# Lennart0HU/Master-Thesis-Deep-Reinforcement-Learning-DDPG-in-Home-Energy-Management

Measured on AMD Instinct MI355X. Metric: env-steps/sec, higher is better.
Workload: dtype f32; 1 GPU; 65536 parallel shems_LU1 envs per GPU, Charger98 synthetic train table (4320 rows), 72-step episodes, mode=train; envs_per_gpu=65536, episode_len=72, mode=train

## Files before the change

### master-thesis-deep-reinforcement-learning-ddpg-in-home-energy-management_amd/csrc/shems_policy.hip

```cpp
#include <hip/hip_runtime.h>

#include <cstdlib>
#include <cstdio>
#include <cstring>
#include <type_traits>

#include "shems_env_dev.h"
#include "shems_internal.h"

namespace shems {

typedef float f32x16 __attribute__((ext_vector_type(16)));
typedef float f32x4 __attribute__((ext_vector_type(4)));
typedef float f32x2 __attribute__((ext_vector_type(2)));
template <int N> struct FVec { typedef float type __attribute__((ext_vector_type(N))); };
template <> struct FVec<1> { typedef float type; };
template <int N> __device__ __forceinline__ float fvec_get(const typename FVec<N>::type &v, int i) { return v[i]; }
template <> __device__ __forceinline__ float fvec_get<1>(const float &v, int) { return v; }

constexpr int kIn = 9, kH1 = SHEMS_L1, kH2 = SHEMS_L2, kOut = 2;

template <int NA> __device__ __forceinline__ int act_col(int nbase, int t, int row) { return nbase + 64 * (t >> 1) + 2 * row + (t & 1); }
template <int NA> __device__ __forceinline__ typename FVec<NA>::type act_load_a(const float *row_at_nbase, int li);
template <> __device__ __forceinline__ FVec<4>::type act_load_a<4>(const float *p, int li)
// ... 666 lines not shown
        constexpr int keep0_ = free_keep<RD>(-1);
        asm volatile("s_waitcnt vmcnt(%0)" ::"n"(keep0_) : "memory");
        __builtin_amdgcn_sched_barrier(0);
    }
    constexpr int kFreeKsteps = (kChunks - 1) * (kKC / 2) + (kH1 - (kChunks - 1) * kKC) / 2;
    AVec af_[3];
    BVec bf_[3];
#pragma unroll
    for (int k0 = 0; k0 < 2; ++k0) {
        af_[k0] = act_load_a<NA>(Wf + (2 * k0 + lh) * 128, li);
        bf_[k0] = *reinterpret_cast<const BVec *>(Hc + TM * li + (2 * k0 + lh) * BM);
    }
    __builtin_amdgcn_sched_barrier(0);
    FREE_CHUNK(0, kKC / 2);  PSTAMP(3); FREE_CHUNK(1, kKC / 2);  FREE_CHUNK(2, kKC / 2);  FREE_CHUNK(3, kKC / 2);
    FREE_CHUNK(4, kKC / 2);  FREE_CHUNK(5, kKC / 2);  FREE_CHUNK(6, kKC / 2);  FREE_CHUNK(7, kKC / 2);
    if constexpr (HR < 256) {
        asm volatile("s_waitcnt lgkmcnt(0)\n\ts_barrier" ::: "memory");
        [[maybe_unused]] RowRegs rr;
        if constexpr (PRE2) act_row_load(tp_at, rr);
        L1_PHASE(HR / 32);
        if constexpr (PRE2) tp.nz = noise_draw(A.p, env0 + (tid & (BM - 1)));
        asm volatile("s_waitcnt lgkmcnt(0)\n\ts_barrier" ::: "memory");
        if constexpr (PRE2) {
            act_row_store(rr, tp);
            tailpre_store(w1 + (tid & (BM - 1)) * kPreDw, tp);
        }
#pragma unroll
        for (int k0 = 0; k0 < 2; ++k0) {
            constexpr int Kp = (kChunks / 2) * (kKC / 2);
            af_[(Kp + k0) % 3] = act_load_a<NA>(Wf + ((kChunks / 2) % RD) * kFreeChunkFloats + (2 * k0 + lh) * 128, li);
            bf_[(Kp + k0) % 3] = *reinterpret_cast<const BVec *>(Hc + TM * li + (2 * k0 + lh) * BM);
        }
        __builtin_amdgcn_sched_barrier(0);
    }
    FREE_CHUNK(8, kKC / 2);  FREE_CHUNK(9, kKC / 2);  FREE_CHUNK(10, kKC / 2); FREE_CHUNK(11, kKC / 2);
    FREE_CHUNK(12, kKC / 2); FREE_CHUNK(13, kKC / 2); FREE_CHUNK(14, kKC / 2);
    PSTAMP(4);
    FREE_CHUNK(15, (kH1 - (kChunks - 1) * kKC) / 2);
    PSTAMP(10);

#pragma unroll
    for (int gl = 0; gl < NA / 2; ++gl)
        act_l3_group<TM, TM == 4 ? 4 : 16>(acc + 2 * gl, tl + kH2P, nbase + 64 * gl, li, lh, RED_OF(nbase / 64 + gl));
    __syncthreads();

    PSTAMP(11);
    double reward = 0.0;
    const int64_t i = env0 + tid;
    if (tid < BM && i < A.m) {
        float p0, p1;
        act_finish(tl, {RED_OF(0), RED_OF(1), RED_OF(2), RED_OF(3)}, {RED_OF(4), RED_OF(5), RED_OF(6), RED_OF(7)}, tid, p0, p1);
        reward = act_env_tail<HP>(A, i, p0, p1, learner, goff, A.obs == A.v.obs ? xR + tid * kIn : nullptr, PRE ? xP + tid * kPreDw : PRE2 ? w1 + tid * kPreDw : nullptr, hp, gx);
    }
    PSTAMP(12);
    act_block_reward<NW>(A, reward, Wc, bid);
}
template <int TM, int NW, int RD>
__global__ __launch_bounds__(64 * NW, NW / 4) void k_act(ActArgs A) { k_act_body<TM, NW, RD, 0>(A, nullptr); }
template <int TM, int NW, int RD>
__global__ __launch_bounds__(64 * NW, NW / 4) void k_act_hp(ActArgs A, const shems_group_hparams *hp) { k_act_body<TM, NW, RD, 1>(A, hp); }
template <int TM, int NW, int RD>
__global__ __launch_bounds__(64 * NW, NW / 4) void k_act_x(ActArgs A, const shems_group_hparams *hp, GroupX gx) { k_act_body<TM, NW, RD, 2>(A, hp, gx); }

constexpr int kGChunkFloats = kKC * 64;
constexpr int kGPieces = 4, kGLastPieces = 3;
constexpr int g_pieces(int ch) { return ch > kChunks - 1 ? 0 : ch == kChunks - 1 ? kGLastPieces : kGPieces; }
template <int RD>
constexpr int g_keep(int c)
{
    int n = 0;
    for (int j = c + 2; j <= c + RD - 1; ++j) n += g_pieces(j);
    return n;
}

struct ActSplit {
    unsigned long long *slot;
};
constexpr unsigned long long kSplitEmpty = ~0ull;

template <int TM, int NW, int RD>
constexpr size_t actg_lds_bytes()
{
    return sizeof(float) * (NW * RD * kGChunkFloats + 16 + 256 * 32 * TM + kW1K * 32 * TM + (kTailFloats + 2) +
                            8 * 32 * TM * kOut + 32 * TM * kIn + 32 * TM * kPreDw + 4);
}

__device__ __forceinline__ void g_piece(const char *sbase, uint32_t voff, uint32_t lds_base, int q)
{
    switch (q) {
    case 0: glds16_asm<-2048>(sbase, voff, lds_base); break;
    case 1: glds16_asm<-1024>(sbase, voff, lds_base); break;
    case 2: glds16_asm<0>(sbase, voff, lds_base); break;
    default: glds16_asm<1024>(sbase, voff, lds_base); break;
    }
}

template <int TM, int NW, int NS, int RD, int HP, bool TILED = false>
__device__ __forceinline__ void k_actg_body(const ActArgs &A, const ActSplit &X, const shems_group_hparams *hp, const GroupX gx = GroupX{nullptr, nullptr})
{
    static_assert(NW * NS == 8 && (NW == 4 || NW == 8), "8 column groups per env tile: 8 waves, or two workgroups of 4");
#ifdef SHEMS_STAMP_ACT
#define GSTAMP(i, cond) do { if (threadIdx.x == 0 && (cond)) { reinterpret_cast<unsigned long long *>(A.block_reward)[2*(i)] = __builtin_amdgcn_s_memtime(); reinterpret_cast<unsigned long long *>(A.block_reward)[2*(i)+1] = __builtin_amdgcn_s_memrealtime(); } } while (0)
#else
#define GSTAMP(i, cond)
#endif
    GSTAMP(0, blockIdx.x == 0);
    static_assert(RD >= 2 && RD <= 4 && TM >= 1 && TM <= 2, "ring of 2..4 chunks; relu(layer 1) fully resident (TM <= 2)");
    constexpr int NT_ = 64 * NW, BM = 32 * TM, HR = 256;
    extern __shared__ __attribute__((aligned(16))) char smem[];
    float *Wc = reinterpret_cast<float *>(smem);
    float *Hc = Wc + NW * RD * kGChunkFloats + 16;
    float *xT = Hc + HR * BM;
    float *tl = xT + kW1K * BM;
    float *red = tl + (kTailFloats + 2);
    float *xR = red + 8 * BM * kOut;
    float *xP = xR + BM * kIn;

    const int tid = threadIdx.x;
    const int lane = tid & 63, wave = __builtin_amdgcn_readfirstlane(tid >> 6);
    const int li = lane & 31, lh = lane >> 5;
    int64_t tile = blockIdx.x;
    int half = 0;
    if constexpr (NS == 2) {
        const unsigned b = blockIdx.x, T = gridDim.x >> 1, full = (T >> 3) << 4;
        if (b < full) { tile = (int64_t)(b >> 4) * 8 + (b & 7); half = (b >> 3) & 1; }
        else { tile = (int64_t)(T >> 3) * 8 + ((b - full) >> 1); half = (b - full) & 1; }
    }
    const int64_t env0 = A.m0 + tile * BM;
    const auto [learner, goff, P, s_min, s_max] = act_who(A, env0);
    const int g = half * NW + wave;
    const int nbase = 64 * g;

    const char *W2g = reinterpret_cast<const char *>(P + kOffW2);
    float *Wg = Wc + wave * (RD * kGChunkFloats);
    const uint32_t ring_lds = lds_addr(Wg) + 2 * 1024;
    constexpr size_t kGTlTile = 4 * 64 * 64 * 4, kGTlP = 2 * 64 * 64 * 4;
    const char *gsbase = TILED ? reinterpret_cast<const char *>(A.w2t) + kGTlP + (size_t)g * kGTlTile : W2g + g * 256;
    uint32_t gvoff[kGPieces];
#pragma unroll
    for (int q = 0; q < kGPieces; ++q)
        gvoff[q] = (uint32_t)((4 * q + (lane >> 4)) * (TILED ? 256 : kH2 * 4) + (lane & 15) * 16 - (q - 2) * 1024);
#define G_CHUNK_OFF(chunk) (TILED ? (size_t)((chunk) >> 2) * (8 * kGTlTile) + (size_t)((chunk) & 3) * (kKC * 256) : (size_t)(chunk) * (kKC * kH2 * 4))
#define G_PIECE(chunk, q)                                                                         \
    g_piece(gsbase + G_CHUNK_OFF(chunk), gvoff[q], ring_lds + ((chunk) % RD) * (kGChunkFloats * 4), (q))
    TailPre tp;
    act_pre_index(A, P, env0 + (tid & (BM - 1)), tp);
    ObsRegs<BM, NT_> xr;
    TlRegs tr;
    act_obs_load(A, s_min, s_max, env0, tid, xr);
    constexpr int kL1PerWave = (8 * TM) / NW;
    static_assert(TM == 1 && (kL1PerWave == 1 || kL1PerWave == 2), "k_actg lays layer 1 down for 32-env tiles");
    float wa_[kL1PerWave][kW1K / 2];
    bool wok_[kL1PerWave];
#pragma unroll
    for (int u = 0; u < kL1PerWave; ++u) {
        const int k = 32 * (wave + NW * u) + li;
        wok_[u] = k < kH1;
#pragma unroll
        for (int s2 = 0; s2 < kW1K / 2; ++s2) {
            const int j = 2 * s2 + lh;
            wa_[u][s2] = P[j * kH1 + min(k, kH1 - 1)];
        }
    }
    act_tl_load(P, tid, tr);
    tp.nz = noise_draw(A.p, env0 + (tid & (BM - 1)));
    RowRegs rr;
    act_row_load(act_row_at(A, P, tp), rr);
    act_obs_store<BM, NT_, true>(A, env0, tid, xr, xT, xR);
    act_tl_store(tid, tr, tl);
    asm volatile("s_waitcnt lgkmcnt(0)\n\ts_barrier" ::: "memory");
    GSTAMP(1, blockIdx.x == 0);
#undef L1_A
#define L1_A(s_, j_, g, which) (wok_[which] ? wa_[which][s_] : 0.0f)
    {
#pragma unroll
        for (int ch = 0; ch < RD - 1; ++ch)
#pragma unroll
            for (int q = 0; q < kGPieces; ++q) G_PIECE(ch, q);
        constexpr int kL1Tiles = 8 * TM;
        if constexpr (kL1Tiles / NW >= 2) {
#pragma unroll
            for (int u = 0; u < kL1Tiles / (2 * NW); ++u) {
                const int t0 = wave + 2 * NW * u, g0 = t0 / TM, b0 = t0 % TM, t1 = t0 + NW, g1 = t1 / TM, b1 = t1 % TM;
                L1_TILE2(g0, b0, Hc + (g0 * 32) * BM + TM * li + b0, g1, b1, Hc + (g1 * 32) * BM + TM * li + b1);
            }
        } else {
            const int g0 = wave / TM, b0 = wave % TM;
            L1_TILE(g0, b0, Hc + (g0 * 32) * BM + TM * li + b0);
        }
        act_row_store(rr, tp);
        tailpre_store(xP + (tid & (BM - 1)) * kPreDw, tp);
    }
    asm volatile("s_waitcnt lgkmcnt(0)\n\ts_barrier" ::: "memory");
    GSTAMP(2, blockIdx.x == 0);

    typedef typename FVec<TM>::type BVec;
    f32x16 acc[2][TM];
#pragma unroll
    for (int a = 0; a < 2; ++a)
#pragma unroll
        for (int r = 0; r < 16; ++r) {
            const float bias = tl[act_col<2>(nbase, a, (r & 3) + 8 * (r >> 2) + 4 * lh)];
#pragma unroll
            for (int b = 0; b < TM; ++b) acc[a][b][r] = bias;
        }
    constexpr int kGKsteps = (kChunks - 1) * (kKC / 2) + (kH1 - (kChunks - 1) * kKC) / 2;
    f32x2 af_[3];
    BVec bf_[3];
#define G_KSTEP(c, ks)                                                                                          \
    do {                                                                                                        \
        const int K_ = 8 * (c) + (ks), K2_ = K_ + 2;                                                            \
        if (K2_ < kGKsteps) {                                                                                   \
            const int c2_ = K2_ >> 3, kr_ = 2 * (K2_ & 7) + lh;                                                 \
            af_[K2_ % 3] = *reinterpret_cast<const f32x2 *>(Wg + (c2_ % RD) * kGChunkFloats + kr_ * 64 + 2 * li); \
            bf_[K2_ % 3] = *reinterpret_cast<const BVec *>(Hc + (c2_ * kKC + kr_) * BM + TM * li);              \
        }                                                                                                       \
        _Pragma("unroll") for (int b = 0; b < TM; ++b)                                                          \
            acc[0][b] = __builtin_amdgcn_mfma_f32_32x32x2f32(af_[K_ % 3][0], fvec_get<TM>(bf_[K_ % 3], b), acc[0][b], 0, 0, 0); \
        _Pragma("unroll") for (int b = 0; b < TM; ++b)                                                          \
            acc[1][b] = __builtin_amdgcn_mfma_f32_32x32x2f32(af_[K_ % 3][1], fvec_get<TM>(bf_[K_ % 3], b), acc[1][b], 0, 0, 0); \
        __builtin_amdgcn_sched_group_barrier(0x008, TM, 0);                                                     \
        __builtin_amdgcn_sched_group_barrier(0x100, 1, 0);                                                      \
        __builtin_amdgcn_sched_group_barrier(0x008, TM, 0);                                                     \
        __builtin_amdgcn_sched_group_barrier(0x100, 1, 0);                                                      \
        __builtin_amdgcn_sched_barrier(0);                                                                      \
        if ((ks) < g_pieces((c) + RD - 1)) { G_PIECE((c) + RD - 1, (ks) < kGPieces ? (ks) : 0); __builtin_amdgcn_sched_barrier(0); } \
    } while (0)
#define G_CHUNK(c, NKS)                                                                                         \
    do {                                                                                                        \
        _Pragma("unroll") for (int ks = 0; ks < ((NKS) < 6 ? (NKS) : 6); ++ks) G_KSTEP(c, ks);                  \
        if ((c) + 1 < kChunks) {                                                                                \
            constexpr int keep_ = g_keep<RD>(c);                                                                \
            asm volatile("s_waitcnt vmcnt(%0)" ::"n"(keep_) : "memory");       \
            __builtin_amdgcn_sched_barrier(0);                                                                  \
        }                                                                                                       \
        _Pragma("unroll") for (int ks = 6; ks < (NKS); ++ks) G_KSTEP(c, ks);                                    \
    } while (0)
    {
        constexpr int keep0_ = g_keep<RD>(-1);
        asm volatile("s_waitcnt vmcnt(%0)" ::"n"(keep0_) : "memory");
        __builtin_amdgcn_sched_barrier(0);
    }
#ifdef SHEMS_STAMP_ACT
    if (lane == 0 && blockIdx.x == 0) reinterpret_cast<unsigned long long *>(A.block_reward)[48 + wave] = __builtin_amdgcn_s_memtime();
#endif
#pragma unroll
    for (int k0 = 0; k0 < 2; ++k0) {
        af_[k0] = *reinterpret_cast<const f32x2 *>(Wg + (2 * k0 + lh) * 64 + 2 * li);
        bf_[k0] = *reinterpret_cast<const BVec *>(Hc + (2 * k0 + lh) * BM + TM * li);
    }
    __builtin_amdgcn_sched_barrier(0);
    G_CHUNK(0, kKC / 2);  GSTAMP(3, blockIdx.x == 0); G_CHUNK(1, kKC / 2);  G_CHUNK(2, kKC / 2);  G_CHUNK(3, kKC / 2);
    G_CHUNK(4, kKC / 2);  G_CHUNK(5, kKC / 2);  G_CHUNK(6, kKC / 2);  G_CHUNK(7, kKC / 2);
    G_CHUNK(8, kKC / 2);  G_CHUNK(9, kKC / 2);  G_CHUNK(10, kKC / 2); G_CHUNK(11, kKC / 2);
    G_CHUNK(12, kKC / 2); G_CHUNK(13, kKC / 2); G_CHUNK(14, kKC / 2);
    GSTAMP(4, blockIdx.x == 0);
    G_CHUNK(15, (kH1 - (kChunks - 1) * kKC) / 2);

    GSTAMP(10, blockIdx.x == 0);
#ifdef SHEMS_STAMP_ACT
    if (lane == 0 && blockIdx.x == 0) reinterpret_cast<unsigned long long *>(A.block_reward)[32 + wave] = __builtin_amdgcn_s_memtime();
#endif
    act_l3_group<TM, 0>(acc, tl + kH2P, nbase, li, lh, red + g * (BM * kOut));
    __syncthreads();
    GSTAMP(8, blockIdx.x == 0);

    double reward = 0.0;
    const int64_t i = env0 + tid;
    bool fin = tid < BM && i < A.m;
    float p0 = 0.0f, p1 = 0.0f;
    if (fin) {
        auto red_g = [red](int q) -> const float * { return red + q * (BM * kOut); };
        if constexpr (NS == 1) {
            act_finish(tl, {red_g(0), red_g(1), red_g(2), red_g(3)}, {red_g(4), red_g(5), red_g(6), red_g(7)}, tid, p0, p1);
        } else {
            const float *const mine4[4] = {red_g(4 * half), red_g(4 * half + 1), red_g(4 * half + 2), red_g(4 * half + 3)};
            float m0 = act_half_sum(mine4, tid, 0), m1 = act_half_sum(mine4, tid, 1);
            unsigned long long mine = ((unsigned long long)__float_as_uint(m1) << 32) | __float_as_uint(m0);
            if (mine == kSplitEmpty) { mine = 0x7FC000007FC00000ull; m0 = m1 = __uint_as_float(0x7FC00000u); }
            unsigned long long *slot = X.slot + tile * BM + tid;
            const unsigned long long got = __hip_atomic_exchange(slot, mine, __ATOMIC_RELAXED, __HIP_MEMORY_SCOPE_AGENT);
            if (got == kSplitEmpty) fin = false;
            else __hip_atomic_store(slot, kSplitEmpty, __ATOMIC_RELAXED, __HIP_MEMORY_SCOPE_AGENT);
            const float o0 = __uint_as_float((uint32_t)got), o1 = __uint_as_float((uint32_t)(got >> 32));
            p0 = act_out(tl, 0, half == 0 ? m0 : o0, half == 0 ? o0 : m0);
            p1 = act_out(tl, 1, half == 0 ? m1 : o1, half == 0 ? o1 : m1);
        }
    }
    GSTAMP(9, blockIdx.x == 0);
    GSTAMP(11, tile == 0 && fin);
    if (fin) reward = act_env_tail<HP>(A, i, p0, p1, learner, goff, A.obs == A.v.obs ? xR + tid * kIn : nullptr, xP + tid * kPreDw, hp, gx);
    GSTAMP(12, tile == 0 && fin);
    if constexpr (NS == 1) act_block_reward<NW>(A, reward, Wc, tile);
}
template <int TM, int NW, int NS, int RD>
__global__ __launch_bounds__(64 * NW) void k_actg(ActArgs A, ActSplit X) { k_actg_body<TM, NW, NS, RD, 0>(A, X, nullptr); }
template <int TM, int NW, int NS, int RD>
__global__ __launch_bounds__(64 * NW) void k_actg_hp(ActArgs A, ActSplit X, const shems_group_hparams *hp) { k_actg_body<TM, NW, NS, RD, 1>(A, X, hp); }
template <int TM, int NW, int NS, int RD>
__global__ __launch_bounds__(64 * NW) void k_actg_x(ActArgs A, ActSplit X, const shems_group_hparams *hp, GroupX gx) { k_actg_body<TM, NW, NS, RD, 2>(A, X, hp, gx); }
template <int TM, int NW, int NS, int RD>
__global__ __launch_bounds__(64 * NW) void k_actg_t(ActArgs A, ActSplit X) { k_actg_body<TM, NW, NS, RD, 0, true>(A, X, nullptr); }

constexpr int k2CR = 4, k2RD = 4, k2CF = k2CR * 128;
constexpr int k2NCH = (kH1 + k2CR - 1) / k2CR;
constexpr int k2_pieces(int ch) { return ch < 0 || ch >= k2NCH ? 0 : ch == k2NCH - 1 ? (kH1 - (k2NCH - 1) * k2CR + 1) / 2 : k2CR / 2; }
constexpr size_t act2_lds_bytes()
{
    return sizeof(float) * (4 * k2RD * k2CF + 16 + 128 * 64 + kW1K * 64 + (kTailFloats + 2) + 64 * kPreDw + 4);
}

__device__ __forceinline__ void k2_piece(const char *sbase, uint32_t voff, uint32_t lds_base, int q)
{
    if (q == 0) glds16_asm<-1024>(sbase, voff, lds_base); else glds16_asm<0>(sbase, voff, lds_base);
}

constexpr size_t k2TlTile = 4 * 64 * 64 * 4, k2TlP = 2 * 64 * 64 * 4;
template <bool TILED> constexpr size_t k2_chunk_off(int ch)
{
    return TILED ? (size_t)(ch >> 4) * (8 * k2TlTile) + (size_t)(ch & 15) * (k2CR * 256) : (size_t)ch * (k2CR * kH2 * 4);
}
template <int HP, bool TILED = false>
__device__ __forceinline__ void k_act2_body(const ActArgs &A, const shems_group_hparams *hp, const GroupX gx = GroupX{nullptr, nullptr})
{
    constexpr int TM = 2, BM = 64, NA = 4, NT_ = 256, HR = 128;
    extern __shared__ __attribute__((aligned(16))) char smem[];
    float *Wc = reinterpret_cast<float *>(smem);
    float *Hc = Wc + 4 * k2RD * k2CF + 16;
    float *xT = Hc + HR * BM;
    float *tl = xT + kW1K * BM;
    float *xP = tl + (kTailFloats + 2);
    const int tid = threadIdx.x;
    const int lane = tid & 63, wave = __builtin_amdgcn_readfirstlane(tid >> 6);
    const int li = lane & 31, lh = lane >> 5;
    int64_t bid = blockIdx.x;
    if (A.gcount > 1 && (gridDim.x & 7) == 0) bid = (int64_t)(blockIdx.x & 7) * (gridDim.x >> 3) + (blockIdx.x >> 3);
    const int64_t env0 = A.m0 + bid * BM;
    const auto [learner, goff, P, s_min, s_max] = act_who(A, env0);
    const int nbase = 128 * wave;

    const char *W2g = reinterpret_cast<const char *>(P + kOffW2);
    float *Wf = Wc + wave * (k2RD * k2CF);
    const uint32_t ring_lds = lds_addr(Wf) + 1024;
    const char *wsbase = TILED ? reinterpret_cast<const char *>(A.w2t) + k2TlP + (size_t)wave * (2 * k2TlTile) : W2g + wave * 512;
    uint32_t wvoff[2];
#pragma unroll
    for (int q = 0; q < 2; ++q)
        wvoff[q] = TILED ? (uint32_t)(((lane & 31) >> 4) * k2TlTile + (lane >> 5) * 256 + (lane & 15) * 16 + q * 512 - (q - 1) * 1024)
                         : (uint32_t)((lane >> 5) * (kH2 * 4) + (lane & 31) * 16 + q * (2 * kH2 * 4) - (q - 1) * 1024);
#define K2_PIECE(chunk, q) k2_piece(wsbase + k2_chunk_off<TILED>(chunk), wvoff[q], ring_lds + ((chunk) % k2RD) * (k2CF * 4), (q))
    TailPre tp;
    act_pre_index(A, P, env0 + (tid & (BM - 1)), tp);
    ObsRegs<BM, NT_> xr;
    TlRegs tr;
    act_obs_load(A, s_min, s_max, env0, tid, xr);
    act_tl_load(P, tid, tr);
#define K2_L1_LOAD(gbase, a0_, a1_, kA_, kB_)                                                     \
    _Pragma("unroll") for (int s_ = 0; s_ < kW1K / 2; ++s_) {                                     \
        const int j_ = 2 * s_ + lh;                                                               \
        a0_[s_] = P[j_ * kH1 + min(kA_, kH1 - 1)];                                                \
        a1_[s_] = P[j_ * kH1 + min(kB_, kH1 - 1)];                                                \
    }
    const int t0 = wave, t1 = wave + 4;
    const int kA0 = 32 * (t0 >> 1) + li, kB0 = 32 * (t1 >> 1) + li;
    float wa0[kW1K / 2], wb0[kW1K / 2];
    K2_L1_LOAD(0, wa0, wb0, kA0, kB0)
    tp.nz = noise_draw(A.p, env0 + (tid & (BM - 1)));
    RowRegs rr;
    act_row_load(act_row_at(A, P, tp), rr);
    act_obs_store<BM, NT_, false>(A, env0, tid, xr, xT, nullptr);
    act_tl_store(tid, tr, tl);
    asm volatile("s_waitcnt lgkmcnt(0)\n\ts_barrier" ::: "memory");
#pragma unroll
    for (int ch = 0; ch < k2RD - 1; ++ch)
#pragma unroll
        for (int q = 0; q < 2; ++q) K2_PIECE(ch, q);

#define K2_L1_PHASE(gbase, a0_, a1_)                                                              \
    do {                                                                                          \
        const int gA_ = (gbase) + (t0 >> 1), bA_ = t0 & 1, gB_ = (gbase) + (t1 >> 1), bB_ = t1 & 1; \
        float c0_[kW1K / 2], c1_[kW1K / 2], z0_[kW1K / 2], z1_[kW1K / 2];                         \
        _Pragma("unroll") for (int s_ = 0; s_ < kW1K / 2; ++s_) {                                 \
            const int j_ = 2 * s_ + lh;                                                           \
            c0_[s_] = xT[j_ * BM + TM * li + bA_];                                                \
            c1_[s_] = xT[j_ * BM + TM * li + bB_];                                                \
            z0_[s_] = 32 * gA_ + li < kH1 ? a0_[s_] : 0.0f;                                       \
            z1_[s_] = 32 * gB_ + li < kH1 ? a1_[s_] : 0.0f;                                       \
        }                                                                                         \
        f32x16 u0_, u1_;                                                                          \
        asm volatile("s_nop 1\n\t"                                                                \
                     "v_mfma_f32_32x32x2_f32 %0, %2, %7, 0\n\t"                                   \
                     "v_mfma_f32_32x32x2_f32 %1, %12, %17, 0\n\t"                                 \
                     "v_mfma_f32_32x32x2_f32 %0, %3, %8, %0\n\t"                                  \
                     "v_mfma_f32_32x32x2_f32 %1, %13, %18, %1\n\t"                                \
                     "v_mfma_f32_32x32x2_f32 %0, %4, %9, %0\n\t"                                  \
                     "v_mfma_f32_32x32x2_f32 %1, %14, %19, %1\n\t"                                \
                     "v_mfma_f32_32x32x2_f32 %0, %5, %10, %0\n\t"                                 \
                     "v_mfma_f32_32x32x2_f32 %1, %15, %20, %1\n\t"                                \
                     "v_mfma_f32_32x32x2_f32 %0, %6, %11, %0\n\t"                                 \
                     "v_mfma_f32_32x32x2_f32 %1, %16, %21, %1\n\t"                                \
                     "s_nop 15\n\ts_nop 7"                                                        \
                     : "=&v"(u0_), "=&v"(u1_)                                                     \
                     : "v"(z0_[0]), "v"(z0_[1]), "v"(z0_[2]), "v"(z0_[3]), "v"(z0_[4]),           \
                       "v"(c0_[0]), "v"(c0_[1]), "v"(c0_[2]), "v"(c0_[3]), "v"(c0_[4]),           \
                       "v"(z1_[0]), "v"(z1_[1]), "v"(z1_[2]), "v"(z1_[3]), "v"(z1_[4]),           \
                       "v"(c1_[0]), "v"(c1_[1]), "v"(c1_[2]), "v"(c1_[3]), "v"(c1_[4]));          \
        float *d0_ = Hc + ((gA_ * 32) % HR) * BM + TM * li + bA_, *d1_ = Hc + ((gB_ * 32) % HR) * BM + TM * li + bB_; \
        _Pragma("unroll") for (int r_ = 0; r_ < 16; ++r_) {                                       \
            d0_[((r_ & 3) + 8 * (r_ >> 2) + 4 * lh) * BM] = fmaxf(u0_[r_], 0.0f);                 \
            d1_[((r_ & 3) + 8 * (r_ >> 2) + 4 * lh) * BM] = fmaxf(u1_[r_], 0.0f);                 \
        }                                                                                         \
    } while (0)
    K2_L1_PHASE(0, wa0, wb0);
    float wa1[kW1K / 2], wb1[kW1K / 2];
    {
        const int kA1 = 128 + kA0, kB1 = 128 + kB0;
        K2_L1_LOAD(4, wa1, wb1, kA1, kB1)
    }
    act_row_store(rr, tp);
    tailpre_store(xP + (tid & (BM - 1)) * kPreDw, tp);
    asm volatile("s_waitcnt lgkmcnt(0)\n\ts_barrier" ::: "memory");

    typedef FVec<NA>::type AVec;
    typedef FVec<TM>::type BVec;
    f32x16 acc[NA][TM];
#pragma unroll
    for (int a = 0; a < NA; ++a)
#pragma unroll
        for (int r = 0; r < 16; ++r) {
            const float bias = tl[act_col<NA>(nbase, a, (r & 3) + 8 * (r >> 2) + 4 * lh)];
#pragma unroll
            for (int b = 0; b < TM; ++b) acc[a][b][r] = bias;
        }
    constexpr int kKsteps = kH1 / 2;
    AVec af_[3];
    BVec bf_[3];
#define K2_KSTEP(K)                                                                                             \
    do {                                                                                                        \
        constexpr int K2_ = (K) + 2, c2_ = K2_ >> 1, klim_ = (K) < 64 ? 64 : kKsteps;                           \
        if (K2_ < klim_) {                                                                                      \
            if ((K2_ & 1) == 0) {                                                                               \
                asm volatile("s_waitcnt vmcnt(%0)" ::"n"(k2_pieces(c2_ + 1)) : "memory");                       \
                __builtin_amdgcn_sched_barrier(0);                                                              \
            }                                                                                                   \
            const int kr_ = 2 * (K2_ & 1) + lh;                                                                 \
            af_[K2_ % 3] = act_load_a<NA>(Wf + (c2_ % k2RD) * k2CF + kr_ * 128, li);                            \
            bf_[K2_ % 3] = *reinterpret_cast<const BVec *>(Hc + ((2 * K2_) % HR + lh) * BM + TM * li);          \
        }                                                                                                       \
        _Pragma("unroll") for (int a = 0; a < NA; ++a)                                                          \
            _Pragma("unroll") for (int b = 0; b < TM; ++b)                                                      \
                acc[a][b] = __builtin_amdgcn_mfma_f32_32x32x2f32(fvec_get<NA>(af_[(K) % 3], a), fvec_get<TM>(bf_[(K) % 3], b), acc[a][b], 0, 0, 0); \
        __builtin_amdgcn_sched_group_barrier(0x008, 2, 0);                                                      \
        __builtin_amdgcn_sched_group_barrier(0x100, 1, 0);                                                      \
        __builtin_amdgcn_sched_group_barrier(0x008, 2, 0);                                                      \
        __builtin_amdgcn_sched_group_barrier(0x100, 1, 0);                                                      \
        __builtin_amdgcn_sched_barrier(0);                                                                      \
        if (((K) & 1) < k2_pieces(((K) >> 1) + k2RD - 1)) { K2_PIECE(((K) >> 1) + k2RD - 1, (K) & 1); __builtin_amdgcn_sched_barrier(0); } \
    } while (0)
#define K2_K4(K) K2_KSTEP(K); K2_KSTEP((K) + 1); K2_KSTEP((K) + 2); K2_KSTEP((K) + 3)
#define K2_K16(K) K2_K4(K); K2_K4((K) + 4); K2_K4((K) + 8); K2_K4((K) + 12)
    asm volatile("s_waitcnt vmcnt(%0)" ::"n"(k2_pieces(1) + k2_pieces(2)) : "memory");
    __builtin_amdgcn_sched_barrier(0);
#pragma unroll
    for (int k0 = 0; k0 < 2; ++k0) {
        af_[k0] = act_load_a<NA>(Wf + (2 * k0 + lh) * 128, li);
        bf_[k0] = *reinterpret_cast<const BVec *>(Hc + (2 * k0 + lh) * BM + TM * li);
    }
    __builtin_amdgcn_sched_barrier(0);
    K2_K16(0); K2_K16(16); K2_K16(32); K2_K16(48);
    asm volatile("s_waitcnt lgkmcnt(0)\n\ts_barrier" ::: "memory");
    K2_L1_PHASE(4, wa1, wb1);
    asm volatile("s_waitcnt lgkmcnt(0)\n\ts_barrier" ::: "memory");
    asm volatile("s_waitcnt vmcnt(%0)" ::"n"(k2_pieces(33) + k2_pieces(34)) : "memory");
    __builtin_amdgcn_sched_barrier(0);
#pragma unroll
    for (int k0 = 0; k0 < 2; ++k0) {
        af_[(64 + k0) % 3] = act_load_a<NA>(Wf + ((32 + (k0 >> 1)) % k2RD) * k2CF + (2 * (k0 & 1) + lh) * 128, li);
        bf_[(64 + k0) % 3] = *reinterpret_cast<const BVec *>(Hc + (2 * k0 + lh) * BM + TM * li);
    }
    __builtin_amdgcn_sched_barrier(0);
    K2_K16(64); K2_K16(80); K2_K16(96); K2_K4(112); K2_K4(116); K2_K4(120); K2_KSTEP(124);

#pragma unroll
    for (int gl = 0; gl < 2; ++gl) act_l3_group<TM, 0>(acc + 2 * gl, tl + kH2P, nbase + 64 * gl, li, lh, Wf + gl * (BM * kOut));
    __syncthreads();
    double reward = 0.0;
    const int64_t i = env0 + tid;
    if (tid < BM && i < A.m) {
        auto red_g = [Wc](int g) -> const float * { return Wc + (g >> 1) * (k2RD * k2CF) + (g & 1) * (BM * kOut); };
        float p0, p1;
        act_finish(tl, {red_g(0), red_g(1), red_g(2), red_g(3)}, {red_g(4), red_g(5), red_g(6), red_g(7)}, tid, p0, p1);
        reward = act_env_tail<HP>(A, i, p0, p1, learner, goff, nullptr, xP + tid * kPreDw, hp, gx);
    }
    act_block_reward<4>(A, reward, Hc, bid);
}
__global__ __launch_bounds__(256, 2) void k_act2(ActArgs A) { k_act2_body<0>(A, nullptr); }
__global__ __launch_bounds__(256, 2) void k_act2_hp(ActArgs A, const shems_group_hparams *hp) { k_act2_body<1>(A, hp); }
__global__ __launch_bounds__(256, 2) void k_act2_x(ActArgs A, const shems_group_hparams *hp, GroupX gx) { k_act2_body<2>(A, hp, gx); }
__global__ __launch_bounds__(256, 2) void k_act2_t(ActArgs A) { k_act2_body<0, true>(A, nullptr); }

template <class... Lead>
struct ActKernels {
    typedef void (*Plain)(Lead...);
    typedef void (*WithHp)(Lead..., const shems_group_hparams *);
    typedef void (*WithX)(Lead..., const shems_group_hparams *, GroupX);
    Plain plain; WithHp with_hp; WithX with_x;
    std::atomic<uint64_t> optin[3];
    char what_attr[3][48], what_launch[3][32];

    ActKernels(const char *name, Plain k, WithHp k_hp, WithX k_x) : plain(k), with_hp(k_hp), with_x(k_x), optin{}
    {
        static const char *const suffix[3] = {"", "_hp", "_x"};
        for (int v = 0; v < 3; ++v) {
            snprintf(what_attr[v], sizeof what_attr[v], "hipFuncSetAttribute(%s%s)", name, suffix[v]);
            snprintf(what_launch[v], sizeof what_launch[v], "%s%s launch", name, suffix[v]);
        }
    }
    int launch(dim3 grid, dim3 block, size_t lds, hipStream_t st, const shems_group_hparams *hp, const GroupX *gx, const Lead &...lead)
    {
        const int v = gx ? 2 : hp ? 1 : 0;
        const void *fn = v == 2 ? reinterpret_cast<const void *>(with_x) : v == 1 ? reinterpret_cast<const void *>(with_hp) : reinterpret_cast<const void *>(plain);
        if (int rc = lds_optin(optin[v], fn, (int)lds, what_attr[v])) return rc;
        if (v == 2) hipLaunchKernelGGL(with_x, grid, block, lds, st, lead..., hp, *gx);
        else if (v == 1) hipLaunchKernelGGL(with_hp, grid, block, lds, st, lead..., hp);
        else hipLaunchKernelGGL(plain, grid, block, lds, st, lead...);
        return hip_ok(hipGetLastError(), what_launch[v]);
    }
};

static int launch_act2(const ActArgs &a, hipStream_t st, const shems_group_hparams *hp = nullptr, const GroupX *gx = nullptr)
{
    constexpr size_t lds = act2_lds_bytes();
    static_assert(lds <= 80 * 1024, "k_act2: two workgroups must fit a CU's 160 KB");
    if (a.w2t) {
        static std::atomic<uint64_t> optin{0};
        if (int rc = lds_optin(optin, reinterpret_cast<const void *>(&k_act2_t), (int)lds, "hipFuncSetAttribute(k_act2_t)")) return rc;
        hipLaunchKernelGGL(k_act2_t, dim3((unsigned)((a.m - a.m0 + 63) / 64)), dim3(256), lds, st, a);
        return hip_ok(hipGetLastError(), "k_act2_t launch");
    }
    static ActKernels<ActArgs> form("k_act2", k_act2, k_act2_hp, k_act2_x);
    return form.launch(dim3((unsigned)((a.m - a.m0 + 63) / 64)), dim3(256), lds, st, hp, gx, a);
}

static int pick_tm(int64_t m, int tm_max = 0)
{
    const int tm = m >= 256 * 128 ? 4 : m >= 256 * 64 ? 2 : 1;
    return tm_max > 0 && tm > tm_max ? tm_max : tm;
}
static int group_tm_max(int64_t envs_per_learner) { return envs_per_learner % 128 == 0 ? 4 : envs_per_learner % 64 == 0 ? 2 : 1; }

template <int TM, int NW, int RD>
static int launch_act(const ActArgs &a, hipStream_t st, const shems_group_hparams *hp = nullptr, const GroupX *gx = nullptr)
{
    constexpr int BM = 32 * TM;
    constexpr size_t lds = act_lds_bytes<TM, NW, RD>();
    static_assert(lds <= 160 * 1024, "k_act: LDS image exceeds 160 KB");
    static ActKernels<ActArgs> form("k_act", k_act<TM, NW, RD>, k_act_hp<TM, NW, RD>, k_act_x<TM, NW, RD>);
    return form.launch(dim3((unsigned)((a.m - a.m0 + BM - 1) / BM)), dim3(64 * NW), lds, st, hp, gx, a);
}

constexpr int kSplitMaxTiles = 512;
static int split_scratch(hipStream_t st, ActSplit *out)
{
    struct Slot { int dev; hipStream_t st; ActSplit x; };
    static Slot slots[32];
    static int nslots = 0;
    static std::atomic_flag lock = ATOMIC_FLAG_INIT;
    int dev = 0;
    if (int rc = hip_ok(hipGetDevice(&dev), "hipGetDevice")) return rc;
    while (lock.test_and_set(std::memory_order_acquire)) {}
    int rc = SHEMS_OK;
    int found = -1;
    for (int i = 0; i < nslots; ++i)
        if (slots[i].dev == dev && slots[i].st == st) { found = i; break; }
    if (found < 0) {
        if (nslots == 32) rc = set_error(SHEMS_ERR_ARG, "k_actg: more than 32 (device, stream) pairs use the column-split form");
        else {
            ActSplit x = {nullptr};
            const size_t bytes = (size_t)kSplitMaxTiles * 64 * sizeof(unsigned long long);
            rc = hip_ok(hipMalloc((void **)&x.slot, bytes), "hipMalloc(split slots)");
            if (!rc) rc = hip_ok(hipMemset(x.slot, 0xFF, bytes), "hipMemset(split slots)");
            if (!rc) { slots[nslots] = Slot{dev, st, x}; found = nslots++; }
        }
    }
    if (!rc) *out = slots[found].x;
    lock.clear(std::memory_order_release);
    return rc;
}

template <int TM, int NW, int NS, int RD>
static int launch_actg(const ActArgs &a, hipStream_t st, const shems_group_hparams *hp = nullptr, const GroupX *gx = nullptr)
{
    constexpr int BM = 32 * TM;
    constexpr size_t lds = actg_lds_bytes<TM, NW, RD>();
    static_assert(lds <= 160 * 1024, "k_actg: LDS image exceeds 160 KB");
    static ActKernels<ActArgs, ActSplit> form("k_actg", k_actg<TM, NW, NS, RD>, k_actg_hp<TM, NW, NS, RD>, k_actg_x<TM, NW, NS, RD>);
    const int64_t tiles = (a.m - a.m0 + BM - 1) / BM;
    ActSplit x = {nullptr};
    if constexpr (NS == 2) {
        if (tiles > kSplitMaxTiles) return set_error(SHEMS_ERR_ARG, "k_actg: %lld env tiles exceed the split form's scratch", (long long)tiles);
        if (split_scratch(st, &x) != SHEMS_OK) {
            return launch_actg<1, 8, 1, RD>(a, st, hp, gx);
        }
    }
    if (a.w2t) {
        static std::atomic<uint64_t> optin{0};
        if (int rc = lds_optin(optin, reinterpret_cast<const void *>(&k_actg_t<TM, NW, NS, RD>), (int)lds, "hipFuncSetAttribute(k_actg_t)")) return rc;
        hipLaunchKernelGGL((k_actg_t<TM, NW, NS, RD>), dim3((unsigned)(tiles * NS)), dim3(64 * NW), lds, st, a, x);
        return hip_ok(hipGetLastError(), "k_actg_t launch");
    }
    return form.launch(dim3((unsigned)(tiles * NS)), dim3(64 * NW), lds, st, hp, gx, a, x);
}

static int act_form() { static const int f = []() { const char *e = getenv("SHEMS_ACT_FORM"); return e ? atoi(e) : -1; }(); return f; }
enum ActForm { kAct2, kAct442, kAct242, kAct142, kAct143, kActg1422, kActg1423, kActg1813 };
static const char *act_form_name(ActForm f)
{
    static const char *const names[] = {"shems::k_act2", "shems::k_act<4, 4, 2>", "shems::k_act<2, 4, 2>", "shems::k_act<1, 4, 2>",
                                        "shems::k_act<1, 4, 3>", "shems::k_actg<1, 4, 2, 2>", "shems::k_actg<1, 4, 2, 3>",
                                        "shems::k_actg<1, 8, 1, 3>"};
    return names[f];
}
static int act_form_tile_envs(ActForm f)
{
    switch (f) {
    case kAct2: return 64;
    case kAct442: return 128;
    case kAct242: return 64;
    default: return 32;
    }
}

static ActForm pick_act_form(int64_t cnt, int tm_max, int gcount, bool w2t, bool want_sum)
{
    const int form = act_form();
    if (w2t && gcount > 0) {
        const int tmt = pick_tm(cnt, tm_max);
        return tmt == 4 ? kAct442 : tmt == 2 ? kAct242 : kAct142;
    }
    if (form < 0 && cnt > 8192 && gcount <= 1) return kAct2;
    if (form == 12 && (tm_max == 0 || tm_max >= 2)) return kAct2;
    const int tm = pick_tm(cnt, tm_max);
    if (tm == 4) return kAct442;
    if (tm == 2) return kAct242;
    if (form == 2) return kAct142;
    if (form == 3) return kAct143;
    const bool split_fits = (cnt + 31) / 32 <= kSplitMaxTiles;
    if ((form == 10 || (form < 0 && cnt > 128 * 32)) && !want_sum && split_fits) return kActg1422;
    if (form == 8 || !split_fits || (form != 9 && (cnt > 128 * 32 || want_sum))) return kActg1813;
    return kActg1423;
}

static int act_tile_envs(int64_t m) { return act_form_tile_envs(pick_act_form(m, 0, 0, false, true)); }

static int dispatch_act(const ActArgs &a, hipStream_t st, const shems_group_hparams *hp = nullptr, const GroupX *gx = nullptr)
{
#ifdef SHEMS_STAMP_ACT
    const bool want_sum = false;
#else
    const bool want_sum = a.block_reward != nullptr;
#endif
    switch (pick_act_form(a.m - a.m0, a.tm_max, a.gcount, a.w2t != nullptr, want_sum)) {
    case kAct2: return launch_act2(a, st, hp, gx);
    case kAct442: return launch_act<4, 4, 2>(a, st, hp, gx);
    case kAct242: return launch_act<2, 4, 2>(a, st, hp, gx);
    case kAct142: return launch_act<1, 4, 2>(a, st, hp, gx);
    case kAct143: return launch_act<1, 4, 3>(a, st, hp, gx);
    case kActg1422: return launch_actg<1, 4, 2, 2>(a, st, hp, gx);
    case kActg1423: return launch_actg<1, 4, 2, 3>(a, st, hp, gx);
    case kActg1813: return launch_actg<1, 8, 1, 3>(a, st, hp, gx);
    }
    return set_error(SHEMS_ERR_ARG, "dispatch_act: no form");
}

__global__ __launch_bounds__(256) void k_act_tail(ActArgs A, const float *__restrict__ part, int n_part, const float *__restrict__ b3)
{
    const int64_t i = (int64_t)blockIdx.x * 256 + threadIdx.x;
    if (i >= A.m) return;
    float p0 = 0.0f, p1 = 0.0f;
    for (int p = 0; p < n_part; ++p) {
        const float2 v = reinterpret_cast<const float2 *>(part)[(int64_t)p * A.m + i];
        p0 += v.x; p1 += v.y;
    }
    act_env_tail(A, i, b3[0] + p0, b3[1] + p1, 0, 0, nullptr);
}

template <int HP>
__device__ __forceinline__ void act_tail_g_body(const ActArgs &A, const float *__restrict__ part, int n_part, const float *__restrict__ b3_0,
                                                const shems_group_hparams *hp, const GroupX gx = GroupX{nullptr, nullptr})
{
    const int64_t i = (int64_t)blockIdx.x * 256 + threadIdx.x;
    if (i >= A.m) return;
    const int64_t learner = i / A.genvs, r = i - learner * A.genvs, goff = learner * A.gstride;
    const float *b3 = gsh(b3_0, goff);
    const float2 *pp = reinterpret_cast<const float2 *>(part) + learner * n_part * A.genvs + r;
    float p0 = 0.0f, p1 = 0.0f;
    for (int p = 0; p < n_part; ++p) {
        const float2 v = pp[(int64_t)p * A.genvs];
        p0 += v.x; p1 += v.y;
    }
    act_env_tail<HP>(A, i, b3[0] + p0, b3[1] + p1, learner, goff, nullptr, nullptr, hp, gx);
}
template <bool HP>
__global__ __launch_bounds__(256) void k_act_tail_g(ActArgs A, const float *__restrict__ part, int n_part, const float *__restrict__ b3_0,
                                                    const shems_group_hparams *hp)
{
    act_tail_g_body<HP ? 1 : 0>(A, part, n_part, b3_0, hp);
}
__global__ __launch_bounds__(256) void k_act_tail_gx(ActArgs A, const float *__restrict__ part, int n_part, const float *__restrict__ b3_0,
                                                     const shems_group_hparams *hp, GroupX gx)
{
    act_tail_g_body<2>(A, part, n_part, b3_0, hp, gx);
}

static int wide_act(const ActArgs &a, int l1, int l2, float *d_ws, hipStream_t st)
{
    if (!d_ws || ((uintptr_t)d_ws & 15) != 0) return set_error(SHEMS_ERR_ARG, "shems_wide_act: 16-byte aligned workspace required");
    float *part = d_ws + wide_act_part_offset(l1, a.m);
    int n_part = 0;
    if (int rc = wide_actor_pre(a.p.actor, a.p.s_min, a.p.s_max, l1, l2, a.obs, a.m, d_ws, part, &n_part, st)) return rc;
    const float *b3 = a.p.actor + ((int64_t)kIn * l1 + l1 + (int64_t)l1 * l2 + l2 + (int64_t)l2 * kOut);
    hipLaunchKernelGGL(k_act_tail, dim3((unsigned)((a.m + 255) / 256)), dim3(256), 0, st, a, part, n_part, b3);
    return hip_ok(hipGetLastError(), "k_act_tail launch");
}

}

using namespace shems;

extern "C" {

int shems_act_step_grid(int64_t n_envs, int64_t *out_blocks)
{
    if (n_envs <= 0 || !out_blocks) return set_error(SHEMS_ERR_ARG, "shems_act_step_grid: bad arguments");
    const int bm = act_tile_envs(n_envs);
    *out_blocks = (n_envs + bm - 1) / bm;
    return SHEMS_OK;
}

int shems_act_step_kernel(int64_t n_envs, int grouped, char *out, int32_t cap)
{
    if (n_envs <= 0 || !out || cap < 2) return set_error(SHEMS_ERR_ARG, "shems_act_step_kernel: bad arguments");
    snprintf(out, (size_t)cap, "%s", act_form_name(pick_act_form(n_envs, 0, grouped ? 2 : 1, grouped == 2, false)));
    return SHEMS_OK;
}

int shems_act_step_group_kernel(int64_t n_envs, int64_t envs_per_learner, int tiled, char *out, int32_t cap)
{
    if (n_envs <= 0 || envs_per_learner < 32 || envs_per_learner % 32 != 0 || n_envs % envs_per_learner != 0 || !out || cap < 2)
        return set_error(SHEMS_ERR_ARG, "shems_act_step_group_kernel: bad arguments");
    const int64_t count = n_envs / envs_per_learner;
    snprintf(out, (size_t)cap, "%s", act_form_name(pick_act_form(n_envs, group_tm_max(envs_per_learner), (int)count, tiled != 0, false)));
    return SHEMS_OK;
}

static int check_act(const shems_act_params *p, const char *fn, shems_group_w2t *tiled = nullptr)
{
    if (!p || !p->actor || !p->s_min || !p->s_max) return set_error(SHEMS_ERR_ARG, "%s: actor / s_min / s_max required", fn);
    if (p->noise_kind < SHEMS_NOISE_GAUSS || p->noise_kind > SHEMS_NOISE_EPS) return set_error(SHEMS_ERR_ARG, "%s: unknown noise_kind %d", fn, p->noise_kind);
    if (p->train && p->noise_kind == SHEMS_NOISE_OU && !p->ou_state) return set_error(SHEMS_ERR_ARG, "%s: OU noise needs ou_state", fn);
    if (((uintptr_t)p->actor & 15) != 0) return set_error(SHEMS_ERR_ARG, "%s: actor parameter block must be 16-byte aligned", fn);
    if (!tiled) return w2t_flux_guard(p->actor, fn);
    if (!w2t_lookup(p->actor, tiled)) *tiled = shems_group_w2t{nullptr, nullptr};
    return SHEMS_OK;
}

static void step_args(ActArgs &a, const shems_view *v, const shems_act_params *p)
{
    std::memset(&a, 0, sizeof a);
    a.v = *v; a.p = *p; a.obs = v->obs; a.m = v->n_envs; a.do_step = 1;
}

static int attach_ring(const char *fn, ActArgs &a, const shems_replay *ring, const shems_ring_window *window, int64_t block_envs)
{
    if (!ring || !window || window->count <= 0) return SHEMS_OK;
    if (ring->capacity <= 0 || !ring->s || !ring->a || !ring->r || !ring->s2 || !ring->done)
        return set_error(SHEMS_ERR_ARG, "%s: incomplete replay ring", fn);
    if (window->count > ring->capacity || window->count > block_envs || window->pos < 0)
        return set_error(SHEMS_ERR_ARG, "%s: ring window larger than the ring or its block of %lld envs", fn, (long long)block_envs);
    if (window->offset < 0 || window->offset >= block_envs)
        return set_error(SHEMS_ERR_ARG, "%s: ring window offset %lld outside its block of %lld envs", fn, (long long)window->offset,
                         (long long)block_envs);
    a.ring = *ring; a.win = *window; a.use_ring = 1;
    return SHEMS_OK;
}

int shems_actor_forward_dev(const shems_act_params *p, const float *d_obs, int64_t m, float *d_a, void *stream)
{
    shems_group_w2t t;
    if (int rc = check_act(p, "shems_actor_forward_dev", &t)) return rc;
    if (!d_obs || !d_a || m <= 0) return set_error(SHEMS_ERR_ARG, "shems_actor_forward_dev: bad buffers");
    ActArgs a;
// ... 172 lines not shown
```

Measured before the change: 401.5 million env-steps/s.

## Load layer-2 weights directly into registers instead of staging through an LDS ring

Replaces the async global-to-LDS ring buffer for W2 chunks, along with its vmcnt waits and the LDS reads back, with direct global loads into a register ring of depth k2AD that is prefetched k2AD k-steps ahead. LDS use falls sharply because only a small reduction scratch area stays, which could allow higher occupancy. The cost is more VGPRs (8 float4 registers in flight) and reliance on per-wave global load latency and L2 hits for the weights, with no LDS-level sharing. PSTAMP timing hooks are also added.

Result: no change. 402.8 million env-steps/s (median of 6 runs) (+0.3%).

```diff
diff --git a/master-thesis-deep-reinforcement-learning-ddpg-in-home-energy-management_amd/csrc/shems_policy.hip b/master-thesis-deep-reinforcement-learning-ddpg-in-home-energy-management_amd/csrc/shems_policy.hip
--- a/master-thesis-deep-reinforcement-learning-ddpg-in-home-energy-management_amd/csrc/shems_policy.hip
+++ b/master-thesis-deep-reinforcement-learning-ddpg-in-home-energy-management_amd/csrc/shems_policy.hip
@@ -992,31 +992,37 @@
 template <int TM, int NW, int NS, int RD>
 __global__ __launch_bounds__(64 * NW) void k_actg_t(ActArgs A, ActSplit X) { k_actg_body<TM, NW, NS, RD, 0, true>(A, X, nullptr); }
 
-constexpr int k2CR = 4, k2RD = 4, k2CF = k2CR * 128;
-constexpr int k2NCH = (kH1 + k2CR - 1) / k2CR;
-constexpr int k2_pieces(int ch) { return ch < 0 || ch >= k2NCH ? 0 : ch == k2NCH - 1 ? (kH1 - (k2NCH - 1) * k2CR + 1) / 2 : k2CR / 2; }
+#ifndef SHEMS_K2_AD
+#define SHEMS_K2_AD 8
+#endif
+constexpr int k2AD = SHEMS_K2_AD;
+constexpr int k2RedFloats = 8 * 64 * kOut;
 constexpr size_t act2_lds_bytes()
 {
-    return sizeof(float) * (4 * k2RD * k2CF + 16 + 128 * 64 + kW1K * 64 + (kTailFloats + 2) + 64 * kPreDw + 4);
-}
-
-__device__ __forceinline__ void k2_piece(const char *sbase, uint32_t voff, uint32_t lds_base, int q)
-{
-    if (q == 0) glds16_asm<-1024>(sbase, voff, lds_base); else glds16_asm<0>(sbase, voff, lds_base);
+    return sizeof(float) * (k2RedFloats + 128 * 64 + kW1K * 64 + (kTailFloats + 2) + 64 * kPreDw + 4);
 }
 
 constexpr size_t k2TlTile = 4 * 64 * 64 * 4, k2TlP = 2 * 64 * 64 * 4;
-template <bool TILED> constexpr size_t k2_chunk_off(int ch)
-{
-    return TILED ? (size_t)(ch >> 4) * (8 * k2TlTile) + (size_t)(ch & 15) * (k2CR * 256) : (size_t)ch * (k2CR * kH2 * 4);
+template <bool TILED> constexpr size_t k2_a_off(int K, int g)
+{
+    return TILED ? (size_t)(K >> 5) * (8 * k2TlTile) + (size_t)g * k2TlTile + (size_t)(K & 31) * 512 : (size_t)K * (2 * kH2 * 4) + (size_t)g * 256;
+}
+template <bool TILED> __device__ __forceinline__ FVec<4>::type k2_a_load(const char *wsbase, uint32_t wvoff, int K)
+{
+    typedef const __attribute__((address_space(1))) f32x2 *GP;
+    uint64_t b0 = reinterpret_cast<uint64_t>(wsbase + k2_a_off<TILED>(K, 0)), b1 = reinterpret_cast<uint64_t>(wsbase + k2_a_off<TILED>(K, 1));
+    asm("" : "+s"(b0));
+    if (TILED) asm("" : "+s"(b1)); else b1 = b0 + (k2_a_off<false>(0, 1) - k2_a_off<false>(0, 0));
+    const f32x2 x = *reinterpret_cast<GP>(b0 + wvoff), y = *reinterpret_cast<GP>(b1 + wvoff);
+    return FVec<4>::type{x[0], x[1], y[0], y[1]};
 }
 template <int HP, bool TILED = false>
 __device__ __forceinline__ void k_act2_body(const ActArgs &A, const shems_group_hparams *hp, const GroupX gx = GroupX{nullptr, nullptr})
 {
     constexpr int TM = 2, BM = 64, NA = 4, NT_ = 256, HR = 128;
     extern __shared__ __attribute__((aligned(16))) char smem[];
-    float *Wc = reinterpret_cast<float *>(smem);
-    float *Hc = Wc + 4 * k2RD * k2CF + 16;
+    float *red = reinterpret_cast<float *>(smem);
+    float *Hc = red + k2RedFloats;
     float *xT = Hc + HR * BM;
     float *tl = xT + kW1K * BM;
     float *xP = tl + (kTailFloats + 2);
@@ -1030,15 +1036,11 @@
     const int nbase = 128 * wave;
 
     const char *W2g = reinterpret_cast<const char *>(P + kOffW2);
-    float *Wf = Wc + wave * (k2RD * k2CF);
-    const uint32_t ring_lds = lds_addr(Wf) + 1024;
     const char *wsbase = TILED ? reinterpret_cast<const char *>(A.w2t) + k2TlP + (size_t)wave * (2 * k2TlTile) : W2g + wave * 512;
-    uint32_t wvoff[2];
-#pragma unroll
-    for (int q = 0; q < 2; ++q)
-        wvoff[q] = TILED ? (uint32_t)(((lane & 31) >> 4) * k2TlTile + (lane >> 5) * 256 + (lane & 15) * 16 + q * 512 - (q - 1) * 1024)
-                         : (uint32_t)((lane >> 5) * (kH2 * 4) + (lane & 31) * 16 + q * (2 * kH2 * 4) - (q - 1) * 1024);
-#define K2_PIECE(chunk, q) k2_piece(wsbase + k2_chunk_off<TILED>(chunk), wvoff[q], ring_lds + ((chunk) % k2RD) * (k2CF * 4), (q))
+    const uint32_t wvoff = (uint32_t)(lh * (TILED ? 256 : kH2 * 4) + li * 8);
+    typedef FVec<NA>::type AVec;
+    AVec aw_[k2AD];
+#define K2_A_LOAD(K) aw_[(K) % k2AD] = k2_a_load<TILED>(wsbase, wvoff, (K))
     TailPre tp;
     act_pre_index(A, P, env0 + (tid & (BM - 1)), tp);
     ObsRegs<BM, NT_> xr;
@@ -1062,9 +1064,7 @@
     act_tl_store(tid, tr, tl);
     asm volatile("s_waitcnt lgkmcnt(0)\n\ts_barrier" ::: "memory");
 #pragma unroll
-    for (int ch = 0; ch < k2RD - 1; ++ch)
-#pragma unroll
-        for (int q = 0; q < 2; ++q) K2_PIECE(ch, q);
+    for (int k0 = 0; k0 < k2AD; ++k0) K2_A_LOAD(k0);
 
 #define K2_L1_PHASE(gbase, a0_, a1_)                                                              \
     do {                                                                                          \
@@ -1111,7 +1111,6 @@
     tailpre_store(xP + (tid & (BM - 1)) * kPreDw, tp);
     asm volatile("s_waitcnt lgkmcnt(0)\n\ts_barrier" ::: "memory");
 
-    typedef FVec<NA>::type AVec;
     typedef FVec<TM>::type BVec;
     f32x16 acc[NA][TM];
 #pragma unroll
@@ -1123,61 +1122,42 @@
             for (int b = 0; b < TM; ++b) acc[a][b][r] = bias;
         }
     constexpr int kKsteps = kH1 / 2;
-    AVec af_[3];
     BVec bf_[3];
 #define K2_KSTEP(K)                                                                                             \
     do {                                                                                                        \
-        constexpr int K2_ = (K) + 2, c2_ = K2_ >> 1, klim_ = (K) < 64 ? 64 : kKsteps;                           \
-        if (K2_ < klim_) {                                                                                      \
-            if ((K2_ & 1) == 0) {                                                                               \
-                asm volatile("s_waitcnt vmcnt(%0)" ::"n"(k2_pieces(c2_ + 1)) : "memory");                       \
-                __builtin_amdgcn_sched_barrier(0);                                                              \
-            }                                                                                                   \
-            const int kr_ = 2 * (K2_ & 1) + lh;                                                                 \
-            af_[K2_ % 3] = act_load_a<NA>(Wf + (c2_ % k2RD) * k2CF + kr_ * 128, li);                            \
-            bf_[K2_ % 3] = *reinterpret_cast<const BVec *>(Hc + ((2 * K2_) % HR + lh) * BM + TM * li);          \
-        }                                                                                                       \
+        constexpr int K2_ = (K) + 2, klim_ = (K) < 64 ? 64 : kKsteps;                                           \
+        if (K2_ < klim_) bf_[K2_ % 3] = *reinterpret_cast<const BVec *>(Hc + ((2 * K2_) % HR + lh) * BM + TM * li); \
         _Pragma("unroll") for (int a = 0; a < NA; ++a)                                                          \
             _Pragma("unroll") for (int b = 0; b < TM; ++b)                                                      \
-                acc[a][b] = __builtin_amdgcn_mfma_f32_32x32x2f32(fvec_get<NA>(af_[(K) % 3], a), fvec_get<TM>(bf_[(K) % 3], b), acc[a][b], 0, 0, 0); \
-        __builtin_amdgcn_sched_group_barrier(0x008, 2, 0);                                                      \
-        __builtin_amdgcn_sched_group_barrier(0x100, 1, 0);                                                      \
+                acc[a][b] = __builtin_amdgcn_mfma_f32_32x32x2f32(fvec_get<NA>(aw_[(K) % k2AD], a), fvec_get<TM>(bf_[(K) % 3], b), acc[a][b], 0, 0, 0); \
         __builtin_amdgcn_sched_group_barrier(0x008, 2, 0);                                                      \
         __builtin_amdgcn_sched_group_barrier(0x100, 1, 0);                                                      \
         __builtin_amdgcn_sched_barrier(0);                                                                      \
-        if (((K) & 1) < k2_pieces(((K) >> 1) + k2RD - 1)) { K2_PIECE(((K) >> 1) + k2RD - 1, (K) & 1); __builtin_amdgcn_sched_barrier(0); } \
+        if ((K) + k2AD < kKsteps) { K2_A_LOAD((K) + k2AD); __builtin_amdgcn_sched_barrier(0); }                 \
     } while (0)
 #define K2_K4(K) K2_KSTEP(K); K2_KSTEP((K) + 1); K2_KSTEP((K) + 2); K2_KSTEP((K) + 3)
 #define K2_K16(K) K2_K4(K); K2_K4((K) + 4); K2_K4((K) + 8); K2_K4((K) + 12)
-    asm volatile("s_waitcnt vmcnt(%0)" ::"n"(k2_pieces(1) + k2_pieces(2)) : "memory");
+#pragma unroll
+    for (int k0 = 0; k0 < 2; ++k0) bf_[k0] = *reinterpret_cast<const BVec *>(Hc + (2 * k0 + lh) * BM + TM * li);
     __builtin_amdgcn_sched_barrier(0);
-#pragma unroll
-    for (int k0 = 0; k0 < 2; ++k0) {
-        af_[k0] = act_load_a<NA>(Wf + (2 * k0 + lh) * 128, li);
-        bf_[k0] = *reinterpret_cast<const BVec *>(Hc + (2 * k0 + lh) * BM + TM * li);
-    }
-    __builtin_amdgcn_sched_barrier(0);
+    PSTAMP(3);
     K2_K16(0); K2_K16(16); K2_K16(32); K2_K16(48);
     asm volatile("s_waitcnt lgkmcnt(0)\n\ts_barrier" ::: "memory");
     K2_L1_PHASE(4, wa1, wb1);
     asm volatile("s_waitcnt lgkmcnt(0)\n\ts_barrier" ::: "memory");
-    asm volatile("s_waitcnt vmcnt(%0)" ::"n"(k2_pieces(33) + k2_pieces(34)) : "memory");
-    __builtin_amdgcn_sched_barrier(0);
-#pragma unroll
-    for (int k0 = 0; k0 < 2; ++k0) {
-        af_[(64 + k0) % 3] = act_load_a<NA>(Wf + ((32 + (k0 >> 1)) % k2RD) * k2CF + (2 * (k0 & 1) + lh) * 128, li);
-        bf_[(64 + k0) % 3] = *reinterpret_cast<const BVec *>(Hc + (2 * k0 + lh) * BM + TM * li);
-    }
+#pragma unroll
+    for (int k0 = 0; k0 < 2; ++k0) bf_[(64 + k0) % 3] = *reinterpret_cast<const BVec *>(Hc + (2 * k0 + lh) * BM + TM * li);
     __builtin_amdgcn_sched_barrier(0);
     K2_K16(64); K2_K16(80); K2_K16(96); K2_K4(112); K2_K4(116); K2_K4(120); K2_KSTEP(124);
-
-#pragma unroll
-    for (int gl = 0; gl < 2; ++gl) act_l3_group<TM, 0>(acc + 2 * gl, tl + kH2P, nbase + 64 * gl, li, lh, Wf + gl * (BM * kOut));
+    PSTAMP(4);
+
+#pragma unroll
+    for (int gl = 0; gl < 2; ++gl) act_l3_group<TM, 0>(acc + 2 * gl, tl + kH2P, nbase + 64 * gl, li, lh, red + (2 * wave + gl) * (BM * kOut));
     __syncthreads();
     double reward = 0.0;
     const int64_t i = env0 + tid;
     if (tid < BM && i < A.m) {
-        auto red_g = [Wc](int g) -> const float * { return Wc + (g >> 1) * (k2RD * k2CF) + (g & 1) * (BM * kOut); };
+        auto red_g = [red](int g) -> const float * { return red + g * (BM * kOut); };
         float p0, p1;
         act_finish(tl, {red_g(0), red_g(1), red_g(2), red_g(3)}, {red_g(4), red_g(5), red_g(6), red_g(7)}, tid, p0, p1);
         reward = act_env_tail<HP>(A, i, p0, p1, learner, goff, nullptr, xP + tid * kPreDw, hp, gx);
```
